# shibiaowan/SHARP

Hardware: AMD Instinct MI355X
Metric: cells/sec end-to-end SHARP (fixed genes, n.RP); ARI vs reference labels (higher is better)
Workload: dtype f64

## Files before the change

### sharp_amd/csrc/common.hpp

```cpp
#pragma once
#include <hip/hip_runtime.h>
#include <functional>

#include <cstdint>
#include <cstdio>
#include <map>
#include <stdexcept>
#include <string>
#include <vector>

#include "../../include/sharp_hip.h"

namespace sharp {

struct Error : std::runtime_error {
    int code;
    Error(int c, const std::string &m) : std::runtime_error(m), code(c) {}
};

void set_error(const std::string &msg);

#define SHARP_HIP_CHECK(expr)                                                                   \
    do {                                                                                        \
        hipError_t _e = (expr);                                                                 \
// ... 37 lines not shown
};

struct Knobs {
    bool rp_dual = true;
    int rp_two_streams = -1;
    int rp_ahead = 2;
    int rp_chunk = 0;
    int rp_cp_wgs = 8;
    int rp_ap_wgs = 4;
    int rp_kernel = 0;
    int rp_pc_wgs = 2;
    int rp_pc_shape = 0;
    int x_storage = 0;
    bool block_prefetch = true;
    bool unlimited_batch = true;
    int unlimited_window_mb = 0;
    int ml_min_levels = 0;
    bool hc_mono = false, hc_seq = false;
    int hc_split = -1;
    int hc_ranges = 0, hc_wpt = 0, hc_finish_at = 15, hc_chunk = 0;
    int tail_threads = 4;
    bool tail_priority = true;
    bool dist_i8 = false;
    bool stats_sums = true;
    bool stats_lane = true;
    bool hc_tri = false;
    bool hc_prep_early = true;
    bool hc_pipe = true;
    bool mean_early = false;
    int gemm_slice = 8;
    bool proj_host = false;
    int hc_front = 0;
    bool hc_nn_gemm = true;
    bool hc_half = false;
    int host_threads = 0;
    int upload_threads = 0;
    std::vector<int> devices;
    int front_overlap = 0;
    int hc_first_chunk = 0;
    int host_group = 1;
    bool decision_log = false;
    bool free_later = true;
    bool step_marks = false;
    int rp_shape = 0;
};
const Knobs &knobs();
void reload_knobs();
// ... 147 lines not shown
```

### sharp_amd/csrc/hclust.hip

```cpp
#include "hclust_task.hpp"

#include <algorithm>
#include <array>
#include <climits>
#include <cmath>
#include <cstring>
#include <limits>

#include "linalg.hpp"

namespace sharp {

namespace {

template <typename T>
struct PinnedBuf {
    T *p = nullptr;
    size_t n = 0;
    PinnedBuf() = default;
    PinnedBuf(const PinnedBuf &) = delete;
    PinnedBuf &operator=(const PinnedBuf &) = delete;
    ~PinnedBuf() { if (p) (void)hipHostFree(p); }
    void ensure(size_t count) {
        if (count <= n) return;
// ... 38 lines not shown
    }
}

inline long long rup(long long v, long long a) { return (v + a - 1) / a * a; }

constexpr int kHcSplitMaxTasks = 136;
constexpr int kMlMinLevels = 256;
static int ml_min_levels() { return knobs().ml_min_levels > 0 ? knobs().ml_min_levels : kMlMinLevels; }
constexpr int kHcSplitMinObs = 1000;

struct ChunkJob {
    size_t i0 = 0, i1 = 0;
    int T = 0, slot = 0;
    bool pipe = false, first = true;
    hipEvent_t input_ready = nullptr;
    bool i8 = false;
    std::vector<HcMeta> metas;
    std::vector<RowPrepTask> prep;
    std::vector<GemmTask> g;
    long long oOut = 0, oM = 0, oLab = 0;
    int max_n = 0, max_p = 0, max_nk = 0, max_kpad = 0, NS = 1;
    bool split = false;
    bool ml = false;
    std::vector<MlMeta> mlmetas;
    int ml_off = 0, ml_cnt = 0, mlt_off = 0, mlt_cnt = 0;
    bool seq_pending = false;
    bool has_next = false;
    bool one_range = false;
    int scratch_slot = 0;
    int prev_slot = 1, next_slot = 1;
    int plan_row = -1;
    int next2_slot = -1;
    hipEvent_t mid_event = nullptr;
    int mid_round = 8;
    bool mid_recorded = false;
    struct Range { int t0, t1; int off[5], cnt[5]; int off8 = 0; bool any_sym, any_feat; };
    std::vector<Range> ranges;
};
enum : int { PH_DIST = 1, PH_AGGLO = 2, PH_STATS = 4, PH_ALL = 7 };
struct PipeEvents {
    hipEvent_t in = nullptr, out[8] = {nullptr}, gemm[6] = {nullptr}, hc[6] = {nullptr}, done[6] = {nullptr}, prep[6] = {nullptr};
};
PipeEvents &pipe_events() {
    PipeEvents &e = per_slot<PipeEvents>();
    if (!e.in) {
        SHARP_HIP_CHECK(hipEventCreateWithFlags(&e.in, hipEventDisableTiming));
// ... 45 lines not shown
            M.kmin = M.kmax = tk.prm.N_cluster;
        } else {
            M.kmin = tk.prm.minN;
            M.kmax = std::min(tk.prm.maxN, tk.n - 1);
            SHARP_REQUIRE(M.kmin >= 2 && M.kmax >= M.kmin, "get_opt_hclust: empty range of cluster numbers (minN.cluster..maxN.cluster)");
        }
        M.nk = M.kmax - M.kmin + 1;
        M.kpad = static_cast<int>(rup(M.kmax, 16));
        M.oD = oD; oD += static_cast<long long>(M.nld) * M.nld;
        M.oD0 = oD0; if (M.symmetric == 1) oD0 += static_cast<long long>(M.nld) * M.nld;
        M.oCr = oCr; if (M.symmetric != 2) oCr += static_cast<long long>(M.n) * M.p;
        M.oCt = oCt; if (M.symmetric != 2) oCt += rup(M.p, 16) * M.nld;
        M.oNrm = oN; oN += M.n;
        M.oM = oM; oM += M.n;
        M.oLab = oLab; oLab += static_cast<long long>(M.nk) * M.n;
        M.oH = M.oT = M.oG = oK; oK += static_cast<long long>(M.nld) * M.kpad;
        M.oCSt = oCS; oCS += static_cast<long long>(M.p) * M.kpad;
        M.oQ = oQ; oQ += static_cast<long long>(M.kpad) * M.kpad;
        M.oOut = oOut; oOut += 2LL * M.nk;
        max_n = std::max(max_n, M.n); max_p = std::max(max_p, M.p); max_nk = std::max(max_nk, M.nk);
        max_kpad = std::max(max_kpad, M.kpad);
    }
    J.oOut = oOut; J.oM = oM; J.oLab = oLab; J.max_n = max_n; J.max_p = max_p; J.max_nk = max_nk; J.max_kpad = max_kpad;
    SHARP_REQUIRE(max_nk > ml_min_levels() ||
                  stats_lds_bytes(max_n, std::max(max_kpad, 64)) <= ST_LDS_MAX,
                  "get_opt_hclust: this many observations with this many candidate cluster numbers does not fit the silhouette kernel "
                  "(LDS: 8 B per observation rounded up to a power of two + 36 B per candidate cluster)");
    { HostTimer ht("hc_workspace_alloc");
    W.D.ensure(oD); W0.S0.ensure(oD); W0.S1.ensure(oD); W.D0.ensure(std::max<long long>(oD0, 1)); W.Cr.ensure(oCr); W.Ct.ensure(oCt); W.nrm.ensure(oN);
    W.height.ensure(oM); W.ia.ensure(oM); W.ib.ensure(oM); W.lab.ensure(oLab);
    W.H.ensure(oK); W.T.ensure(oK); W.G.ensure(oK); W.CSt.ensure(oCS); W.Q.ensure(oQ); W.out.ensure(oOut); }
    { HostTimer ht("hc_workspace_alloc");
    W.meta.ensure(T); W.prep.ensure(T); W.gemm.ensure(5 * static_cast<size_t>(T)); W.status.ensure(T); }
    {
        bool parts = knobs().hc_nn_gemm;
#ifdef SHARP_LAB
        if (knobs().dist_i8 && max_p <= 8192) parts = false;
#endif
        long long oNN = 0;
        if (parts) for (int t = 0; t < T; ++t) if (!metas[t].symmetric && metas[t].nld <= 2048) oNN += static_cast<long long>(metas[t].nld / 128) * metas[t].nld;
        if (oNN > 0) {
            W.nnp.ensure(oNN);
            oNN = 0;
            for (int t = 0; t < T; ++t) if (!metas[t].symmetric && metas[t].nld <= 2048) { metas[t].nn = W.nnp.p + oNN; oNN += static_cast<long long>(metas[t].nld / 128) * metas[t].nld; }
        }
    }
    W.meta.upload(metas.data(), T);

    int NS = T >= 194 ? 2 : 1;
    {
        const bool split = knobs().hc_split >= 0 ? knobs().hc_split == 1 : (T <= kHcSplitMaxTasks && max_n >= kHcSplitMinObs);
        J.split = split;
        if (!knobs().hc_seq && ((!knobs().hc_mono && split) || max_n > HR_MAXN)) NS = 1;
    }
    if (knobs().hc_ranges > 0) NS = std::max(1, std::min(8, knobs().hc_ranges));
    if (J.pipe || J.one_range) NS = 1;
    if (J.max_nk > ml_min_levels()) NS = 1;
    NS = std::min(NS, T);
    std::vector<RowPrepTask> &prep = J.prep;
    prep.assign(T, RowPrepTask());
    for (int t = 0; t < T; ++t) {
        const HcTask &tk = tasks[i0 + t];
        const HcMeta &M = metas[t];
        prep[t] = RowPrepTask{tk.d_mat, tk.ld, M.n, M.p, M.nld, static_cast<int>(rup(M.p, 16)), M.symmetric, W.Cr.p + M.oCr,
                              W.Ct.p + M.oCt, W.nrm.p + M.oNrm, W.D.p + M.oD};
    }
    W.prep.upload(prep.data(), T);
    typedef ChunkJob::Range Range;
    J.NS = NS;
    std::vector<Range> &ranges = J.ranges;
    ranges.assign(NS, Range());
    std::vector<GemmTask> &g = J.g;
    g.clear();
    g.reserve(5 * static_cast<size_t>(T));
    for (int s = 0; s < NS; ++s) {
        Range &R = ranges[s];
        R.t0 = static_cast<int>(static_cast<long long>(T) * s / NS);
        R.t1 = static_cast<int>(static_cast<long long>(T) * (s + 1) / NS);
        R.any_sym = R.any_feat = false;
        for (int kind = 0; kind < 5; ++kind) {
            R.off[kind] = static_cast<int>(g.size());
            for (int t = R.t0; t < R.t1; ++t) {
                const HcMeta &M = metas[t];
                R.any_sym |= M.symmetric != 0; R.any_feat |= M.symmetric == 0;
                switch (kind) {
                    case 0:
                        if (!M.symmetric) g.push_back(GemmTask{W.Ct.p + M.oCt, W.Ct.p + M.oCt, W.D.p + M.oD, M.n, M.n, M.p, M.nld, M.nld, M.nld, 1, 1, 1,
                                                               const_cast<double *>(M.nn), M.method == 8});
                        break;
                    case 1:
                        g.push_back(GemmTask{W.Cr.p + M.oCr, W.H.p + M.oH, W.CSt.p + M.oCSt, M.p, M.kpad, M.n, M.p, M.kpad, M.kpad, 0, 0, 0});
                        break;
                    case 2:
                        g.push_back(GemmTask{W.CSt.p + M.oCSt, W.Ct.p + M.oCt, W.G.p + M.oG, M.kpad, M.n, M.p, M.kpad, M.nld, M.nld, 0, 0, 0});
                        break;
                    case 3:
                        g.push_back(GemmTask{W.CSt.p + M.oCSt, W.CSt.p + M.oCSt, W.Q.p + M.oQ, M.kpad, M.kpad, M.p, M.kpad, M.kpad, M.kpad, 0, 0, 0});
                        break;
                    default:
                        if (M.symmetric == 1) g.push_back(GemmTask{W.H.p + M.oH, W.D0.p + M.oD0, W.T.p + M.oT, M.kpad, M.n, M.n, M.kpad, M.nld, M.nld, 0, 0, 0});
                        break;
                }
            }
            R.cnt[kind] = static_cast<int>(g.size()) - R.off[kind];
        }
    }
#ifdef SHARP_LAB
    J.i8 = knobs().dist_i8 && max_p <= 8192;
    if (J.i8) {
        std::vector<DistI8Task> d8;
        size_t oSl = 0, oSc = 0;
        for (int t = 0; t < T; ++t) if (!metas[t].symmetric) { oSl += dist_i8_slice_bytes(metas[t].nld, metas[t].p); oSc += metas[t].nld; }
        W.sl.ensure(std::max<size_t>(oSl, 1)); W.slscale.ensure(std::max<size_t>(oSc, 1));
        oSl = 0; oSc = 0;
        for (int s = 0; s < NS; ++s) {
            ranges[s].off8 = static_cast<int>(d8.size());
            for (int t = ranges[s].t0; t < ranges[s].t1; ++t) {
                const HcMeta &M = metas[t];
                if (M.symmetric) continue;
                d8.push_back(DistI8Task{W.Cr.p + M.oCr, W.D.p + M.oD, W.sl.p + oSl, W.slscale.p + oSc, M.n, M.p, M.nld, (M.p + 31) / 32});
                oSl += dist_i8_slice_bytes(M.nld, M.p); oSc += M.nld;
            }
        }
        W.i8.ensure(std::max<size_t>(d8.size(), 1));
        if (!d8.empty()) W.i8.upload(d8.data(), d8.size());
    }
#endif
    J.ml = max_nk > ml_min_levels();
    if (J.ml) {
        SHARP_REQUIRE(static_cast<size_t>(max_kpad) * 22 + 64 <= HR_LDS_CU, "get_opt_hclust: too many candidate cluster numbers (more than ~7400)");
        J.ml_off = static_cast<int>(g.size());
        for (int t = 0; t < T; ++t) {
            const HcMeta &M = metas[t];
            g.push_back(GemmTask{W.Ct.p + M.oCt, W.CSt.p + M.oCSt, W.G.p + M.oG, M.n, M.kpad, M.p, M.nld, M.kpad, M.kpad, 0, 0, 0});
        }
        J.ml_cnt = T;
        J.mlt_off = static_cast<int>(g.size());
        for (int t = 0; t < T; ++t) {
            const HcMeta &M = metas[t];
            if (M.symmetric == 1) g.push_back(GemmTask{W.D0.p + M.oD0, W.H.p + M.oH, W.T.p + M.oT, M.n, M.kpad, M.n, M.nld, M.kpad, M.kpad, 0, 0, 0});
        }
        J.mlt_cnt = static_cast<int>(g.size()) - J.mlt_off;
        W.gemm.ensure(g.size());
        J.mlmetas.assign(T, MlMeta());
        long long oS = 0, oMg = 0, oFin = 0;
        for (int t = 0; t < T; ++t) {
            const HcMeta &M = metas[t];
            J.mlmetas[t].oS = oS; oS += 2LL * M.n * M.nk;
            J.mlmetas[t].oMerge = oMg; oMg += M.nk;
            J.mlmetas[t].oFin = oFin; oFin += M.kmax;
        }
// ... 51 lines not shown
        }
        if (phases & PH_AGGLO) {
        if (J.pipe && !J.first) SHARP_HIP_CHECK(hipStreamWaitEvent(st, EV.hc[J.prev_slot], 0));
        {
            const bool use_rnn = !knobs().hc_seq;
            KernelTimer tm("hclust");
            HcAggloDid did;
            if (use_rnn && hclust_bulk_synchronous(agglo, J.split, W0.img, W0.remaining, J.mid_event, J.mid_round, &did)) J.mid_recorded = true;
            if (!use_rnn || !(J.pipe && J.has_next)) launch_sequential(use_rnn);
            else J.seq_pending = true;
            if (J.plan_row >= 0 && s == 0) {
                std::array<int, kHcPlanCols> &row = batch_plan().rows[J.plan_row];
                row[9] = J.seq_pending; row[10] = did.form; row[14] = did.wpt; row[15] = did.finish_at;
            }
        }
        if (J.pipe) SHARP_HIP_CHECK(hipEventRecord(EV.hc[J.slot], st));
        if (J.pipe && knobs().step_marks)
            SHARP_HIP_CHECK(hipLaunchHostFunc(st, [](void *) { step_mark("    (device) an agglomeration ends"); }, nullptr));
        }
        if (!(phases & PH_STATS)) continue;
        if (J.pipe && J.has_next) SHARP_HIP_CHECK(hipStreamWaitEvent(st, EV.gemm[J.next_slot], 0));
        if (J.pipe && J.next2_slot >= 0) SHARP_HIP_CHECK(hipStreamWaitEvent(st, EV.gemm[J.next2_slot], 0));
        if (J.seq_pending) { launch_sequential(true); J.seq_pending = false; }
        const HcStatsRange stats{dmeta, Ts, max_n, max_p, J.max_nk, max_kpad, R.any_sym, W.gemm.p, R.off, R.cnt, W.ia.p, W.ib.p, W.lab.p,
                                 W.H.p, W.Cr.p, W.CSt.p, W.T.p, W.G.p, W.Q.p, W.nrm.p, W.out.p};
        const HcManyLevels many{&J.metas, &J.mlmetas, W.mlmeta.p, J.oM, J.ml_off, J.ml_cnt, J.mlt_off, J.mlt_cnt, W.mlr1.p, W.mlr2.p, W.mlcntF.p,
                                W.mlcn2m.p, W.mlB.p, W.mlcn2F.p, W.mltot2.p, W.mlS.p};
        hclust_level_stats(stats, J.ml ? &many : nullptr);
        if (NS > 1) {
            SHARP_HIP_CHECK(hipEventRecord(ev_out[s], st));
            SHARP_HIP_CHECK(hipStreamWaitEvent(main_stream, ev_out[s], 0));
        }
    }
    if (J.pipe && (phases & PH_STATS)) SHARP_HIP_CHECK(hipEventRecord(EV.done[J.slot], chunk_stream));
    if (J.pipe && (phases & PH_STATS) && knobs().step_marks)
        SHARP_HIP_CHECK(hipLaunchHostFunc(chunk_stream, [](void *) { step_mark("    (device) a chunk's statistics end"); }, nullptr));
}

void finish_chunk(const std::vector<HcTask> &tasks, ChunkJob &J, bool want_v, std::vector<HcResult> &out, bool want_status) {
    Ctx &c = ctx();
    Workspace &W = ws(J.slot);
    const size_t i0 = J.i0;
    const int T = J.T;
    const long long oOut = J.oOut, oM = J.oM, oLab = J.oLab;
    const std::vector<HcMeta> &metas = J.metas;
    if (J.pipe) SHARP_HIP_CHECK(hipStreamWaitEvent(c.stream, pipe_events().done[J.slot], 0));
    W.h_out.ensure(std::max<long long>(oOut, 1)); W.h_height.ensure(std::max<long long>(oM, 1));
    double *h_out = W.h_out.p, *h_height = W.h_height.p;
// ... 476 lines not shown
```

### sharp_amd/csrc/hclust_stats.hip

```cpp
#include "hclust_task.hpp"

#include <algorithm>
#include <vector>

#include "linalg.hpp"

namespace sharp {

__global__ __launch_bounds__(HC_THREADS) void cutree_kernel(const HcMeta *__restrict__ metas, const int *__restrict__ ia_all,
                                                            const int *__restrict__ ib_all, int *__restrict__ lab_all) {
    const HcMeta M = metas[blockIdx.x];
    const int n = M.n;
    const int *ia = ia_all + M.oM, *ib = ib_all + M.oM;
    int *lab = lab_all + M.oLab;
    extern __shared__ __attribute__((aligned(16))) unsigned char sm[];
    unsigned char *lds_cursor = sm;
    CUTREE_ARRAYS(LDS_CARVE, n)
    const int tid = threadIdx.x;
    for (int i = tid; i < n; i += HC_THREADS) { absorbed[i] = 0x7fffffff; parent[i] = static_cast<uint16_t>(i); }
    __syncthreads();
    for (int s = tid; s < n - 1; s += HC_THREADS) { absorbed[ib[s] - 1] = s; parent[ib[s] - 1] = static_cast<uint16_t>(ia[s] - 1); }
    __syncthreads();
    const int chunk = (n + HC_THREADS - 1) / HC_THREADS;
    for (int L = 0; L < M.nk; ++L) {
// ... 50 lines not shown
    const double *Cr = Cr_all + M.oCr;
    const int j = j0 + lane;
    const bool live = j < p;
    double *mine = acc + static_cast<size_t>(wave) * kpad * 64 + lane;
    int i = wave;
    for (; i + 3 * SS_WAVES < n; i += 4 * SS_WAVES) {
        double x[4];
        int c[4];
#pragma unroll
        for (int u = 0; u < 4; ++u) {
            c[u] = __builtin_amdgcn_readfirstlane(lab[i + u * SS_WAVES]) - 1;
            x[u] = live ? Cr[static_cast<long long>(i + u * SS_WAVES) * p + j] : 0.0;
        }
#pragma unroll
        for (int u = 0; u < 4; ++u) mine[c[u] * 64] += x[u];
    }
    for (; i < n; i += SS_WAVES) {
        const int c = __builtin_amdgcn_readfirstlane(lab[i]) - 1;
        mine[c * 64] += live ? Cr[static_cast<long long>(i) * p + j] : 0.0;
    }
    __syncthreads();
    double *CSt = CSt_all + M.oCSt;
    for (int q = tid; q < kpad * 64; q += 64 * SS_WAVES) {
        const int c = q >> 6, l = q & 63;
        if (j0 + l >= p) continue;
        double v = acc[c * 64 + l];
#pragma unroll
        for (int w = 1; w < SS_WAVES; ++w) v += acc[(w * kpad + c) * 64 + l];
        CSt[static_cast<long long>(j0 + l) * kpad + c] = v;
    }
}

__global__ void copy_d_kernel(const HcMeta *__restrict__ metas, const double *__restrict__ Dall, double *__restrict__ D0all) {
    const HcMeta M = metas[blockIdx.y];
    if (M.symmetric != 1) return;
    const long long tot = static_cast<long long>(M.n) * M.nld;
    const double *D = Dall + M.oD;
    double *D0 = D0all + M.oD0;
    for (long long q = blockIdx.x * static_cast<long long>(blockDim.x) + threadIdx.x; q < tot;
         q += static_cast<long long>(gridDim.x) * blockDim.x)
        D0[q] = D[q];
}


__global__ __launch_bounds__(ST_THREADS) void stats_kernel(const HcMeta *__restrict__ metas, const int *__restrict__ lab_all,
                                                           const double *__restrict__ T_all, const double *__restrict__ G_all,
// ... 390 lines not shown
    allow_dynamic_lds(ml_level_kernel, lds_l);
    for (int t = 0; t < T; ++t) {
        const HcMeta &M = metas[t];
        const int blocks = std::min((M.n + ML_WAVES - 1) / ML_WAVES, c.num_cu * std::max(1, static_cast<int>(HR_LDS_CU / std::max<size_t>(lds_c, 1))));
        hipLaunchKernelGGL(ml_cells_kernel, dim3(blocks), dim3(64 * ML_WAVES), lds_c, st, r.metas, ml.dml, t, r.lab, r.T, r.G, r.nrm,
                           ml.r1, ml.r2, ml.cn2m, ml.cntF, ml.cn2F, ml.S);
        hipLaunchKernelGGL(ml_level_kernel, dim3(M.nk), dim3(ST_THREADS), lds_l, st, r.metas, ml.dml, t, ml.S, ml.B, r.out);
    }
    launch_check("ml_cells_kernel");
}

}

void hclust_level_stats(const HcStatsRange &r, const HcManyLevels *ml) {
    hipStream_t st = ctx().stream;
    const int Ts = r.tasks, max_n = r.max_n, max_p = r.max_p, max_nk = r.max_nk, max_kpad = r.max_kpad;
    {
        const size_t lds = cutree_lds_bytes(max_n);
        allow_dynamic_lds(cutree_kernel, lds);
        KernelTimer tm("cutree");
        hipLaunchKernelGGL(cutree_kernel, dim3(Ts), dim3(HC_THREADS), lds, st, r.metas, r.ia, r.ib, r.lab);
        launch_check("cutree_kernel");
    }
    const bool sums = knobs().stats_sums && !ml && max_kpad <= SS_KMAX;
    if (!sums || r.any_sym) {
        KernelTimer tm("onehot");
        hipLaunchKernelGGL(onehot_kernel, dim3(64, Ts), dim3(256), 0, st, r.metas, r.lab, r.H);
        launch_check("onehot_kernel");
    }
    if (sums) {
        KernelTimer tm("cluster_sums_gemm");
        const size_t lds = cluster_sums_lds_bytes(max_kpad);
        allow_dynamic_lds(cluster_sums_kernel, lds);
        hipLaunchKernelGGL(cluster_sums_kernel, dim3((max_p + 63) / 64, Ts), dim3(64 * SS_WAVES), lds, st, r.metas, r.lab, r.Cr, r.CSt);
        launch_check("cluster_sums_kernel");
    } else if (r.cnt[1]) gemm_tn_f64_batched(r.gemm + r.off[1], r.cnt[1], max_p, max_kpad, "cluster_sums_gemm");
    if (ml) { many_levels_stats(r, *ml); return; }
    if (r.cnt[2]) gemm_tn_f64_batched(r.gemm + r.off[2], r.cnt[2], max_kpad, max_n, "row_cluster_dot_gemm");
    if (r.cnt[3]) gemm_tn_f64_batched(r.gemm + r.off[3], r.cnt[3], max_kpad, max_kpad, "cluster_gram_gemm");
    if (r.cnt[4]) gemm_tn_f64_batched(r.gemm + r.off[4], r.cnt[4], max_kpad, max_n, "dist_cluster_sums_gemm");
    const int kcap = std::max(max_kpad, 64);
    const bool lane_form = knobs().stats_lane && max_kpad <= 64;
    const size_t lds = lane_form ? stats_lane_lds_bytes(max_n, kcap) : stats_lds_bytes(max_n, kcap);
    const auto kern = lane_form ? stats_lane_kernel : stats_kernel;
    allow_dynamic_lds(kern, lds);
    KernelTimer tm("sil_ch_stats");
    const long long blocks = static_cast<long long>((Ts + 7) / 8) * 8 * max_nk;
    hipLaunchKernelGGL(kern, dim3(static_cast<unsigned>(blocks)), dim3(ST_THREADS), lds, st, r.metas, r.lab, r.T,
                       r.G, r.Q, r.nrm, r.out, Ts, max_nk, kcap);
    launch_check("stats_kernel");
}

}
// ... 1 lines not shown
```

### sharp_amd/csrc/hclust_task.hpp

```cpp
#pragma once
#include <algorithm>

#include "hclust.hpp"

namespace sharp {

#define SHARP_HC_LOCAL __attribute__((visibility("hidden")))

struct HcMeta {
    int n, p, nld, kmin, kmax, nk, kpad, method;
    int symmetric, pad0;
    long long oD, oD0;
    long long oCr, oCt, oNrm;
    long long oM;
    long long oLab;
    long long oH, oT, oG;
    long long oCSt, oQ;
    long long oOut;
    const double *nn;
};
struct MlMeta {
    long long oS;
    long long oMerge;
    long long oFin;
};

constexpr int HC_THREADS = 512;
constexpr double HC_INF = 1.0e300;
constexpr int HR_MAXN = 4096;
constexpr size_t HR_LDS_CU = 160 * 1024;
constexpr int ST_THREADS = 512;
constexpr size_t ST_LDS_MAX = 160 * 1024;
constexpr int SS_WAVES = 2, SS_KMAX = 144;
constexpr int ML_WAVES = 3;

template <typename K>
static inline void allow_dynamic_lds(K kern, size_t bytes) {
    SHARP_HIP_CHECK(hipFuncSetAttribute(reinterpret_cast<const void *>(kern), hipFuncAttributeMaxDynamicSharedMemorySize, static_cast<int>(bytes)));
}

__host__ __device__ inline int hc_npow2(int n) { int p = 1; while (p < n) p <<= 1; return p; }

#define LDS_CARVE(type, name, count) \
    [[maybe_unused]] type *name = reinterpret_cast<type *>(lds_cursor); lds_cursor = reinterpret_cast<unsigned char *>(name + (count));
#define LDS_COUNT(type, name, count) lds_bytes += sizeof(type) * static_cast<size_t>(count);

#define HC_SEQ_STATE_ARRAYS(X, n, nal)                                                                                      \
    X(double, disnn, nal)                                                                                                   \
    X(double, pv, 32)                                                                                                       \
    X(int, nn, nal)                                                                                                         \
    X(int, membr, nal)                                                                                                      \
    X(int, list, nal)                                                                                                       \
    X(int, pi, 32)                                                                                                          \
    X(int, cnt, 2)                                                                                                          \
    X(unsigned char, flag, n)
#define HC_SEQ_SCRATCH_ARRAYS(X, n)                                                                                         \
// ... 25 lines not shown
    X(int, wsum, (nwave) + 1)                                                                                               \
    X(unsigned char, tie, nal)
inline size_t hr_image_bytes(int max_n) {
    const int nal = (max_n + 3) & ~3;
    size_t lds_bytes = 0;
    HR_STATE_ARRAYS(LDS_COUNT, nal, 1024 / 64)
    const size_t slack = 64;
    return std::max((lds_bytes + slack + 15) / 16 * 16, static_cast<size_t>(hc_npow2(max_n - 1)) * 16);
}

#define CUTREE_ARRAYS(X, n)                                                                                                 \
    X(int, absorbed, n)                                             \
    X(int, wsum, HC_THREADS / 64 + 1)                                                                                       \
    X(uint16_t, parent, n)                                                                      \
    X(uint16_t, rank, n)
inline size_t cutree_lds_bytes(int max_n) {
    size_t lds_bytes = 0;
    CUTREE_ARRAYS(LDS_COUNT, max_n)
    return lds_bytes + 16;
}

inline size_t cluster_sums_lds_bytes(int kpad) { return static_cast<size_t>(SS_WAVES) * kpad * 64 * 8; }

inline size_t stats_lds_bytes(int max_n, int kcap) {
    int npow2 = 1; while (npow2 < max_n) npow2 <<= 1;
    return static_cast<size_t>(npow2) * 8 + ST_THREADS * 8 + 2 * static_cast<size_t>(kcap) * 8 + (5 * static_cast<size_t>(kcap) + 8) * 4;
}

#define ML_PREP_ARRAYS(X, kf)                                                                                               \
    X(double, cn2, kf)                                                                                                      \
    X(double, ctot, kf)                                                                                                     \
    X(double, part, 1024)                                                                                                   \
    X(int, cnt, kf)
inline size_t ml_prep_lds_bytes(int kpad) {
    size_t lds_bytes = 0;
    ML_PREP_ARRAYS(LDS_COUNT, kpad)
    return lds_bytes + 64;
}

#define ML_CELLS_ARRAYS(X, kf)                                                                                              \
    X(double, st, kf)                        \
    X(double, sg, kf)                                                         \
    X(uint16_t, cnt, kf)                                                                                                    \
    X(uint16_t, live, kf)                                                 \
    X(uint16_t, pos, kf)
__host__ __device__ inline size_t ml_cells_wave_bytes(int kf) {
// ... 15 lines not shown

struct HcAggloRange {
    const HcMeta *metas;
    int tasks, max_n;
    double *D, *S0, *S1;
    int *ia, *ib;
    double *height;
    int *status;
};
struct HcAggloDid {
    int form = 0;
    int wpt = 0;
    int finish_at = 0;
};
SHARP_HC_LOCAL bool hclust_bulk_synchronous(const HcAggloRange &r, bool split, DevBuf<unsigned char> &img, DevBuf<int> &remaining,
                                            hipEvent_t mid_event, int mid_round, HcAggloDid *did = nullptr);
SHARP_HC_LOCAL void hclust_sequential(const HcAggloRange &r, const int *only_if, unsigned char *gstate);

struct GemmTask;
struct HcStatsRange {
    const HcMeta *metas;
    int tasks, max_n, max_p, max_nk, max_kpad;
    bool any_sym;
    const GemmTask *gemm;
    const int *off, *cnt;
    const int *ia, *ib;
    int *lab;
    double *H, *Cr, *CSt, *T, *G, *Q, *nrm, *out;
};
struct HcManyLevels {
    const std::vector<HcMeta> *metas;
    const std::vector<MlMeta> *mlmetas;
    const MlMeta *dml;
    long long oM;
    int ml_off, ml_cnt, mlt_off, mlt_cnt;
    int *r1, *r2, *cntF;
    double *cn2m, *B, *cn2F, *tot2, *S;
};
SHARP_HC_LOCAL void hclust_copy_d(const HcMeta *metas, int tasks, const double *D, double *D0);
SHARP_HC_LOCAL void hclust_level_stats(const HcStatsRange &r, const HcManyLevels *ml);
SHARP_HC_LOCAL void hclust_pack_labels(const HcMeta *metas, int tasks, const int *lab, const int *chosen, const long long *dst_off, int *dst);

SHARP_HC_LOCAL void select_level(const HcParams &prm, int n, int nk, const double *msil, const double *CH, const double *height,
                                 int &oind, int &branch, int &rc);
SHARP_HC_LOCAL double host_ch_euclid(const double *y, int n, int p, const int *cl, int g);

}
```

### sharp_amd/csrc/linalg.hip

```cpp
#include "linalg.hpp"
#include "graph.hpp"

#include <algorithm>
#include <cstring>
#include <string>
#include <type_traits>
#include <vector>

namespace sharp {

typedef __attribute__((address_space(1))) const double *gcdp;
typedef __attribute__((address_space(1))) double *gdp;


typedef double v4f64 __attribute__((ext_vector_type(4)));

__device__ __forceinline__ void lds_barrier() { asm volatile("s_waitcnt lgkmcnt(0)\n\ts_barrier" ::: "memory"); }

constexpr int GT = 64, GK = 16, GLD = 80;

__global__ __launch_bounds__(256) void gemm_tn_f64_kernel(const GemmTask *__restrict__ tasks) {
    const GemmTask t = tasks[blockIdx.z];
    const int m0 = blockIdx.y * GT, n0 = blockIdx.x * GT;
    if (m0 >= t.M || n0 >= t.N) return;
// ... 252 lines not shown
    for (int z0 = 0; z0 < count; z0 += 65535) {
        const int nz = std::min(65535, count - z0);
        if (fast) {
            const int ntm = (max_M + FT - 1) / FT, ntn = (max_N + FT - 1) / FT;
            const int tiles_max = symmetric ? ntn * (ntn + 1) / 2 : ntm * ntn;
            const long long blocks = static_cast<long long>((nz + 7) / 8) * 8 * tiles_max;
            long long slice = blocks;
            if (c.polite) {
                const int per_cu = knobs().gemm_slice;
                if (per_cu > 0) slice = static_cast<long long>(c.num_cu) * per_cu;
            }
            for (long long b0 = 0; b0 < blocks; b0 += slice)
                hipLaunchKernelGGL(gemm_tn_f64_fast_kernel, dim3(static_cast<unsigned>(std::min(slice, blocks - b0))), dim3(512), 0, c.stream,
                                   d_tasks + z0, nz, tiles_max, b0);
        }
        else
            hipLaunchKernelGGL(gemm_tn_f64_kernel, dim3((max_N + GT - 1) / GT, (max_M + GT - 1) / GT, nz), dim3(256), 0, c.stream,
                               d_tasks + z0);
        launch_check("gemm_tn_f64_kernel");
    }
}

constexpr int RP_MAXV = 8;

__device__ __forceinline__ bool fused_rows(const RowPrepTask &t) { return t.mode == 0 && t.p <= 64 * RP_MAXV; }

__global__ __launch_bounds__(256) void row_prep_kernel(const RowPrepTask *__restrict__ tasks, int skip_fused) {
    const RowPrepTask t = tasks[blockIdx.y];
    const int lane = threadIdx.x & 63;
    const int row = blockIdx.x * 4 + (threadIdx.x >> 6);
    if (row >= t.n) return;
    gcdp x = (gcdp)t.src + static_cast<long long>(row) * t.lds;
    gdp cr = (gdp)t.Cr + static_cast<long long>(row) * t.p;
    const int p = t.p;
    if (fused_rows(t) && skip_fused) return;
    if (t.mode == 2) {
        gdp drow = (gdp)t.D + static_cast<long long>(row) * t.nld;
        for (int q = lane; q < p; q += 64) drow[q] = q == row ? 0.0 : x[q];
        return;
    }
    if (t.mode == 0 && p <= 64 * RP_MAXV) {
        double xv[RP_MAXV];
#pragma unroll
        for (int u = 0; u < RP_MAXV; ++u) { const int q = lane + 64 * u; xv[u] = x[q < p ? q : 0]; }
        double s = 0.0;
#pragma unroll
// ... 61 lines not shown
    __syncthreads();
    for (int j = ty; j < 32; j += 8) {
        const int q = q0 + j, r = r0 + tx;
        if (q < t.p_pad && r < t.nld) ((gdp)t.Ct)[static_cast<long long>(q) * t.nld + r] = (r < t.n && q < t.p) ? tile[tx][j] : 0.0;
    }
}

constexpr int RT_ROWS = 16;
__global__ __launch_bounds__(256) void row_prep_t_kernel(const RowPrepTask *__restrict__ tasks) {
    const RowPrepTask t = tasks[blockIdx.y];
    const int r0 = blockIdx.x * RT_ROWS;
    if (!fused_rows(t) || r0 >= t.nld) return;
    extern __shared__ double rt_tile[];
    const int p = t.p, ldt = t.p_pad + 1;
    const int lane = threadIdx.x & 63, wave = threadIdx.x >> 6;
    for (int i = wave; i < RT_ROWS; i += 4) {
        const int row = r0 + i;
        double *trow = rt_tile + i * ldt;
        if (row >= t.n) {
            for (int q = lane; q < t.p_pad; q += 64) trow[q] = 0.0;
            continue;
        }
        gcdp x = (gcdp)t.src + static_cast<long long>(row) * t.lds;
        gdp cr = (gdp)t.Cr + static_cast<long long>(row) * t.p;
        double xv[RP_MAXV];
#pragma unroll
        for (int u = 0; u < RP_MAXV; ++u) { const int q = lane + 64 * u; xv[u] = x[q < p ? q : 0]; }
        double s = 0.0;
#pragma unroll
        for (int u = 0; u < RP_MAXV; ++u) if (lane + 64 * u < p) s += xv[u];
        const double mean = wave_sum(s) / p;
        double ss = 0.0;
#pragma unroll
        for (int u = 0; u < RP_MAXV; ++u) if (lane + 64 * u < p) { const double c = xv[u] - mean; ss += c * c; }
        const double sd = sqrt(wave_sum(ss) / static_cast<double>(p - 1 > 1 ? p - 1 : 1));
        double s2 = 0.0;
#pragma unroll
        for (int u = 0; u < RP_MAXV; ++u) if (lane + 64 * u < p) { xv[u] = (xv[u] - mean) / sd; s2 += xv[u]; }
        const double mean2 = wave_sum(s2) / p;
        double n2 = 0.0;
#pragma unroll
        for (int u = 0; u < RP_MAXV; ++u) if (lane + 64 * u < p) { xv[u] -= mean2; n2 += xv[u] * xv[u]; }
        const double nr = sqrt(wave_sum(n2));
#pragma unroll
        for (int u = 0; u < RP_MAXV; ++u) {
            const int q = lane + 64 * u;
            if (q < p) { const double v = xv[u] / nr; cr[q] = v; trow[q] = v; }
            else if (q < t.p_pad) trow[q] = 0.0;
        }
        if (lane == 0) ((gdp)t.nrm)[row] = 1.0;
    }
    __syncthreads();
    const int i = threadIdx.x & (RT_ROWS - 1);
    for (int q = threadIdx.x / RT_ROWS; q < t.p_pad; q += 256 / RT_ROWS)
        ((gdp)t.Ct)[static_cast<long long>(q) * t.nld + r0 + i] = rt_tile[i * ldt + q];
}

void row_prep_batched(const RowPrepTask *d_tasks, int count, int max_n, int max_p, bool all_feature_rows) {
    if (count <= 0 || max_n <= 0) return;
    Ctx &c = ctx();
    KernelTimer tm("row_prep");
    const bool fused = max_p <= 64 * RP_MAXV;
    for (int z0 = 0; z0 < count; z0 += 65535) {
        const int nz = std::min(65535, count - z0);
        const int nld_max = (max_n + 127) / 128 * 128;
        if (fused) {
            const size_t lds = static_cast<size_t>(RT_ROWS) * ((max_p + 15) / 16 * 16 + 1) * sizeof(double);
            SHARP_HIP_CHECK(hipFuncSetAttribute(reinterpret_cast<const void *>(row_prep_t_kernel), hipFuncAttributeMaxDynamicSharedMemorySize,
                                                static_cast<int>(lds)));
            hipLaunchKernelGGL(row_prep_t_kernel, dim3(nld_max / RT_ROWS, nz), dim3(256), lds, c.stream, d_tasks + z0);
// ... 174 lines not shown
```

### sharp_amd/csrc/linalg.hpp

```cpp
#pragma once
#include "common.hpp"

namespace sharp {

struct GemmTask {
    const double *At;
    const double *Bt;
    double *C;
    int M, N, K;
    long long lda, ldb, ldc;
    int epilogue;
    int symmetric;
    int fast;
    double *nn = nullptr;
    int nn_square = 0;
};

void gemm_tn_f64_batched(const GemmTask *d_tasks, int count, int max_M, int max_N, const char *timer_name, bool fast = false,
                         bool symmetric = false);

struct RowPrepTask {
    const double *src;
    long long lds;
    int n, p, nld;
    int p_pad;
    int mode;
    double *Cr;
    double *Ct;
    double *nrm;
    double *D;
};
void row_prep_batched(const RowPrepTask *d_tasks, int count, int max_n, int max_p, bool all_feature_rows = false);


#ifdef SHARP_LAB
constexpr int kDistI8Slices = 7;
struct DistI8Task {
    const double *Cr;
    double *D;
    signed char *sl;
    double *scale;
    int n, p, nld, ksteps;
};
size_t dist_i8_slice_bytes(int nld, int p);
void dist_i8_batched(const DistI8Task *d_tasks, int count, int max_n);
void dist_i8_slices(const DistI8Task *d_tasks, int count, int max_n);
void dist_i8_products(const DistI8Task *d_tasks, int count, int max_n);
#endif

}
```

### sharp_amd/csrc/runtime.hip

```cpp
#include <cstring>
#include <ctime>
#include <atomic>
#include <condition_variable>
#include <exception>
#include <pthread.h>
#include <mutex>
#include <thread>
#include <unistd.h>
#include <sstream>
#include <tuple>
#include <vector>
#include <cstdio>

#include "common.hpp"

namespace sharp {

static thread_local std::string g_last_error;
static thread_local int t_slot = 0;
static Ctx g_ctxs[kMaxSlots];

void set_error(const std::string &msg) { g_last_error = msg; }

int cur_slot() { return t_slot; }
// ... 269 lines not shown
    auto num = [&](const char *name, int dflt) { const char *e = env(name); return e && *e ? atoi(e) : dflt; };
    if (const char *kv = env("SHARP_RP_KERNEL")) v.rp_kernel = !strcmp(kv, "fused") ? 1 : !strcmp(kv, "dense") ? 2 : !strcmp(kv, "pc") ? 4 : 0;
    if (const char *xs = env("SHARP_X_STORAGE")) v.x_storage = !strcmp(xs, "fp32") ? 32 : !strcmp(xs, "fp64") ? 64 : 0;
    v.host_threads = num("SHARP_HOST_THREADS", 0);
    v.upload_threads = num("SHARP_UPLOAD_THREADS", 0);
    v.tail_threads = num("SHARP_TAIL_THREADS", 4);
    v.unlimited_batch = num("SHARP_UNLIMITED_BATCH", 1) != 0;
    v.unlimited_window_mb = num("SHARP_UNLIMITED_WINDOW_MB", 0);
    v.block_prefetch = num("SHARP_NO_BLOCK_PREFETCH", 0) == 0;
    v.decision_log = num("SHARP_DECISION_LOG", 0) != 0;
    v.host_group = num("SHARP_HOST_GROUP", 1);
    v.step_marks = num("SHARP_STEP_MARKS", 0) != 0;
    v.hc_seq = num("SHARP_HC_SEQ", 0) == 1;
    v.hc_mono = num("SHARP_HC_MONO", 0) == 1;
    v.hc_split = num("SHARP_HC_SPLIT", -1);
    v.hc_pipe = num("SHARP_HC_PIPE", 1) != 0;
    v.hc_chunk = num("SHARP_HC_CHUNK", 0);
    v.hc_first_chunk = num("SHARP_HC_FIRST_CHUNK", 0);
    v.hc_ranges = num("SHARP_HC_RANGES", 0);
    v.hc_wpt = num("SHARP_HC_WPT", 0);
    v.hc_finish_at = num("SHARP_HC_FINISH_AT", 15);
    v.hc_nn_gemm = num("SHARP_HC_NN_GEMM", 1) != 0;
    v.stats_lane = num("SHARP_STATS_LANE", 1) != 0;
    v.ml_min_levels = num("SHARP_ML_MIN_LEVELS", 0);
    v.proj_host = num("SHARP_PROJ_HOST", 0) == 1;
    v.rp_pc_wgs = std::max(1, num("SHARP_RP_PC_WGS", 2));
    v.gemm_slice = num("SHARP_GEMM_SLICE", 8);
#ifdef SHARP_LAB
    if (const char *kv = env("SHARP_RP_KERNEL")) { if (!strcmp(kv, "sparse")) v.rp_kernel = 3; else if (!strcmp(kv, "split")) v.rp_kernel = 5; }
    v.rp_dual = num("SHARP_RP_DUAL", 1) != 0;
    { const int ser = num("SHARP_RP_SERIAL", -1); v.rp_two_streams = ser < 0 ? -1 : (ser == 0 ? 1 : 0); }
    v.rp_chunk = num("SHARP_RP_CHUNK", 0);
    v.rp_ahead = num("SHARP_RP_AHEAD", 2);
    v.rp_cp_wgs = std::max(1, num("SHARP_RP_CP_WGS", 8));
    v.rp_ap_wgs = std::max(1, num("SHARP_RP_AP_WGS", 4));
    v.rp_shape = num("SHARP_RP_SHAPE", 0);
    if (const char *ps = env("SHARP_RP_PC_SHAPE")) v.rp_pc_shape = (*ps == 'a' || *ps == 'A') ? 1 : (*ps == 'b' || *ps == 'B') ? 2 : 0;
    v.mean_early = num("SHARP_MEAN_EARLY", 0) != 0;
    v.hc_prep_early = num("SHARP_HC_PREP_EARLY", 1) != 0;
    v.hc_tri = num("SHARP_HC_TRI", 0) != 0;
    v.hc_front = num("SHARP_HC_FRONT", 0);
    v.hc_half = num("SHARP_HC_HALF", 0) != 0;
    v.stats_sums = num("SHARP_STATS_SUMS", 1) != 0;
    v.dist_i8 = num("SHARP_DIST_I8", 0) != 0;
    v.free_later = num("SHARP_FREE_LATER", 1) != 0;
    v.front_overlap = num("SHARP_FRONT_OVERLAP", 0);
    v.tail_priority = num("SHARP_TAIL_PRIORITY", 1) != 0;
#endif
    if (const char *dl = env("SHARP_DEVICES")) {
        for (const char *q = dl; *q;) {
            char *end = nullptr;
            const long dvc = strtol(q, &end, 10);
            if (end == q) break;
            v.devices.push_back(static_cast<int>(dvc));
            q = *end == ',' ? end + 1 : end;
        }
    }
    return v;
}
static Knobs &knobs_storage() { static Knobs k = read_knobs(); return k; }
const Knobs &knobs() { return knobs_storage(); }
void reload_knobs() { knobs_storage() = read_knobs(); }

namespace {
struct StepMarks { std::mutex mu; std::vector<std::tuple<const char *, int, double>> v; };
StepMarks &step_marks() { static StepMarks *M = new StepMarks; return *M; }
// ... 211 lines not shown
```

Measured before the change: 3.170 million.

## Compute cluster sums from transposed Ct and drop the Cr row buffer

Adds a cluster-sums kernel that reads the transposed normalized matrix Ct through a register-prefetched LDS tile, instead of reading the row-major Cr copy. When no other consumer needs Cr (non-symmetric, small p), row prep no longer writes Cr and its workspace is not allocated. The aim is to cut one full matrix write and its memory footprint. The cost is a more complex kernel with LDS carving and a per-label conditional accumulation that may be slower than the previous reduction.

```diff
diff --git a/sharp_amd/csrc/common.hpp b/sharp_amd/csrc/common.hpp
--- a/sharp_amd/csrc/common.hpp
+++ b/sharp_amd/csrc/common.hpp
@@ -83,7 +83,7 @@
     int tail_threads = 4;
     bool tail_priority = true;
     bool dist_i8 = false;
-    bool stats_sums = true;
+    int stats_sums = 1;
     bool stats_lane = true;
     bool hc_tri = false;
     bool hc_prep_early = true;
diff --git a/sharp_amd/csrc/hclust.hip b/sharp_amd/csrc/hclust.hip
--- a/sharp_amd/csrc/hclust.hip
+++ b/sharp_amd/csrc/hclust.hip
@@ -84,6 +84,8 @@
     int max_n = 0, max_p = 0, max_nk = 0, max_kpad = 0, NS = 1;
     bool split = false;
     bool ml = false;
+    int sums_form = SUMS_CT;
+    bool keep_cr = true;
     std::vector<MlMeta> mlmetas;
     int ml_off = 0, ml_cnt = 0, mlt_off = 0, mlt_cnt = 0;
     bool seq_pending = false;
@@ -175,12 +177,20 @@
         max_kpad = std::max(max_kpad, M.kpad);
     }
     J.oOut = oOut; J.oM = oM; J.oLab = oLab; J.max_n = max_n; J.max_p = max_p; J.max_nk = max_nk; J.max_kpad = max_kpad;
+    J.ml = max_nk > ml_min_levels();
+    J.sums_form = cluster_sums_form(knobs().stats_sums, J.ml, max_n, max_kpad);
+    J.keep_cr = J.sums_form != SUMS_CT;
+    for (const HcMeta &M : metas) J.keep_cr |= M.symmetric != 0 || M.p > kRowPrepFusedMaxP;
+#ifdef SHARP_LAB
+    J.keep_cr |= knobs().dist_i8 && max_p <= 8192;
+#endif
+    if (!J.keep_cr) { oCr = 0; for (HcMeta &M : metas) M.oCr = 0; }
     SHARP_REQUIRE(max_nk > ml_min_levels() ||
                   stats_lds_bytes(max_n, std::max(max_kpad, 64)) <= ST_LDS_MAX,
                   "get_opt_hclust: this many observations with this many candidate cluster numbers does not fit the silhouette kernel "
                   "(LDS: 8 B per observation rounded up to a power of two + 36 B per candidate cluster)");
     { HostTimer ht("hc_workspace_alloc");
-    W.D.ensure(oD); W0.S0.ensure(oD); W0.S1.ensure(oD); W.D0.ensure(std::max<long long>(oD0, 1)); W.Cr.ensure(oCr); W.Ct.ensure(oCt); W.nrm.ensure(oN);
+    W.D.ensure(oD); W0.S0.ensure(oD); W0.S1.ensure(oD); W.D0.ensure(std::max<long long>(oD0, 1)); if (J.keep_cr) W.Cr.ensure(oCr); W.Ct.ensure(oCt); W.nrm.ensure(oN);
     W.height.ensure(oM); W.ia.ensure(oM); W.ib.ensure(oM); W.lab.ensure(oLab);
     W.H.ensure(oK); W.T.ensure(oK); W.G.ensure(oK); W.CSt.ensure(oCS); W.Q.ensure(oQ); W.out.ensure(oOut); }
     { HostTimer ht("hc_workspace_alloc");
@@ -212,10 +222,11 @@
     NS = std::min(NS, T);
     std::vector<RowPrepTask> &prep = J.prep;
     prep.assign(T, RowPrepTask());
+    double *const Cr = J.keep_cr ? W.Cr.p : nullptr;
     for (int t = 0; t < T; ++t) {
         const HcTask &tk = tasks[i0 + t];
         const HcMeta &M = metas[t];
-        prep[t] = RowPrepTask{tk.d_mat, tk.ld, M.n, M.p, M.nld, static_cast<int>(rup(M.p, 16)), M.symmetric, W.Cr.p + M.oCr,
+        prep[t] = RowPrepTask{tk.d_mat, tk.ld, M.n, M.p, M.nld, static_cast<int>(rup(M.p, 16)), M.symmetric, Cr ? Cr + M.oCr : nullptr,
                               W.Ct.p + M.oCt, W.nrm.p + M.oNrm, W.D.p + M.oD};
     }
     W.prep.upload(prep.data(), T);
@@ -242,7 +253,7 @@
                                                                const_cast<double *>(M.nn), M.method == 8});
                         break;
                     case 1:
-                        g.push_back(GemmTask{W.Cr.p + M.oCr, W.H.p + M.oH, W.CSt.p + M.oCSt, M.p, M.kpad, M.n, M.p, M.kpad, M.kpad, 0, 0, 0});
+                        g.push_back(GemmTask{Cr ? Cr + M.oCr : nullptr, W.H.p + M.oH, W.CSt.p + M.oCSt, M.p, M.kpad, M.n, M.p, M.kpad, M.kpad, 0, 0, 0});
                         break;
                     case 2:
                         g.push_back(GemmTask{W.CSt.p + M.oCSt, W.Ct.p + M.oCt, W.G.p + M.oG, M.kpad, M.n, M.p, M.kpad, M.nld, M.nld, 0, 0, 0});
@@ -279,7 +290,6 @@
         if (!d8.empty()) W.i8.upload(d8.data(), d8.size());
     }
 #endif
-    J.ml = max_nk > ml_min_levels();
     if (J.ml) {
         SHARP_REQUIRE(static_cast<size_t>(max_kpad) * 22 + 64 <= HR_LDS_CU, "get_opt_hclust: too many candidate cluster numbers (more than ~7400)");
         J.ml_off = static_cast<int>(g.size());
@@ -377,8 +387,8 @@
         if (J.pipe && J.has_next) SHARP_HIP_CHECK(hipStreamWaitEvent(st, EV.gemm[J.next_slot], 0));
         if (J.pipe && J.next2_slot >= 0) SHARP_HIP_CHECK(hipStreamWaitEvent(st, EV.gemm[J.next2_slot], 0));
         if (J.seq_pending) { launch_sequential(true); J.seq_pending = false; }
-        const HcStatsRange stats{dmeta, Ts, max_n, max_p, J.max_nk, max_kpad, R.any_sym, W.gemm.p, R.off, R.cnt, W.ia.p, W.ib.p, W.lab.p,
-                                 W.H.p, W.Cr.p, W.CSt.p, W.T.p, W.G.p, W.Q.p, W.nrm.p, W.out.p};
+        const HcStatsRange stats{dmeta, Ts, max_n, max_p, J.max_nk, max_kpad, R.any_sym, J.sums_form, W.gemm.p, R.off, R.cnt, W.ia.p, W.ib.p, W.lab.p,
+                                 W.H.p, J.keep_cr ? W.Cr.p : nullptr, W.Ct.p, W.CSt.p, W.T.p, W.G.p, W.Q.p, W.nrm.p, W.out.p};
         const HcManyLevels many{&J.metas, &J.mlmetas, W.mlmeta.p, J.oM, J.ml_off, J.ml_cnt, J.mlt_off, J.mlt_cnt, W.mlr1.p, W.mlr2.p, W.mlcntF.p,
                                 W.mlcn2m.p, W.mlB.p, W.mlcn2F.p, W.mltot2.p, W.mlS.p};
         hclust_level_stats(stats, J.ml ? &many : nullptr);
diff --git a/sharp_amd/csrc/hclust_stats.hip b/sharp_amd/csrc/hclust_stats.hip
--- a/sharp_amd/csrc/hclust_stats.hip
+++ b/sharp_amd/csrc/hclust_stats.hip
@@ -96,6 +96,77 @@
     __syncthreads();
     double *CSt = CSt_all + M.oCSt;
     for (int q = tid; q < kpad * 64; q += 64 * SS_WAVES) {
+        const int c = q >> 6, l = q & 63;
+        if (j0 + l >= p) continue;
+        double v = acc[c * 64 + l];
+#pragma unroll
+        for (int w = 1; w < SS_WAVES; ++w) v += acc[(w * kpad + c) * 64 + l];
+        CSt[static_cast<long long>(j0 + l) * kpad + c] = v;
+    }
+}
+
+__device__ __forceinline__ void sc_lds_barrier() { asm volatile("s_waitcnt lgkmcnt(0)\n\ts_barrier" ::: "memory"); }
+
+typedef double sc_v2f64 __attribute__((ext_vector_type(2)));
+__global__ __launch_bounds__(SC_THREADS) void cluster_sums_ct_kernel(const HcMeta *__restrict__ metas, const int *__restrict__ lab_all,
+                                                                     const double *__restrict__ Ct_all, double *__restrict__ CSt_all) {
+    static_assert(SS_WAVES == 2 && SC_THREADS == 256 && SC_TI == 32 && SS_KMAX <= 256, "the thread maps below");
+    const HcMeta M = metas[blockIdx.y];
+    const int j0 = blockIdx.x * 64;
+    if (j0 >= M.p) return;
+    const int kpad = M.kpad, n = M.n, p = M.p;
+    extern __shared__ __attribute__((aligned(16))) unsigned char sc_sm[];
+    unsigned char *lds_cursor = sc_sm;
+    CLUSTER_SUMS_CT_ARRAYS(LDS_CARVE, kpad, n)
+    const int tid = threadIdx.x, lane = tid & 63;
+    const int wave = __builtin_amdgcn_readfirstlane(tid >> 6);
+    for (int q = tid; q < SS_WAVES * kpad * 64; q += SC_THREADS) acc[q] = 0.0;
+    const int *lab = lab_all + M.oLab + static_cast<long long>(M.nk - 1) * n;
+    for (int i = tid; i < n; i += SC_THREADS) labs[i] = static_cast<unsigned char>(lab[i] - 1);
+    const int ip = tid & 15, jr = tid >> 4;
+    const int ntiles = (n + SC_TI - 1) / SC_TI;
+    const double *Ct = Ct_all + M.oCt + static_cast<long long>(j0 + jr) * M.nld + 2 * ip;
+    const long long row16 = 16LL * M.nld;
+    sc_v2f64 buf[SC_DEPTH][4];
+    auto fetch = [&](sc_v2f64 (&b)[4], int t) {
+#pragma unroll
+        for (int u = 0; u < 4; ++u) {
+            const bool in = t < ntiles && j0 + jr + 16 * u < p;
+            b[u] = in ? *reinterpret_cast<const sc_v2f64 *>(Ct + u * row16 + t * SC_TI) : sc_v2f64{0.0, 0.0};
+        }
+    };
+#pragma unroll
+    for (int d = 0; d < SC_DEPTH; ++d) fetch(buf[d], d);
+    const int cls = wave & 1, csel = wave >> 1;
+    double *mine = acc + static_cast<size_t>(cls) * kpad * 64 + lane;
+    for (int t0 = 0; t0 < ntiles; t0 += SC_DEPTH) {
+#pragma unroll
+        for (int d = 0; d < SC_DEPTH; ++d) {
+            const int t = t0 + d;
+            if (t >= ntiles) break;
+#pragma unroll
+            for (int u = 0; u < 4; ++u) {
+                tile[(2 * ip) * SC_LDT + jr + 16 * u] = buf[d][u].x;
+                tile[(2 * ip + 1) * SC_LDT + jr + 16 * u] = buf[d][u].y;
+            }
+            fetch(buf[d], t + SC_DEPTH);
+            sc_lds_barrier();
+            double x[SC_TI / 2];
+            int c[SC_TI / 2];
+#pragma unroll
+            for (int u = 0; u < SC_TI / 2; ++u) {
+                const int ii = cls + 2 * u, i = t * SC_TI + ii;
+                x[u] = tile[ii * SC_LDT + lane];
+                c[u] = i < n ? __builtin_amdgcn_readfirstlane(static_cast<int>(labs[i])) : -1;
+            }
+#pragma unroll
+            for (int u = 0; u < SC_TI / 2; ++u)
+                if (c[u] >= 0 && (c[u] & 1) == csel) mine[c[u] * 64] += x[u];
+            sc_lds_barrier();
+        }
+    }
+    double *CSt = CSt_all + M.oCSt;
+    for (int q = tid; q < kpad * 64; q += SC_THREADS) {
         const int c = q >> 6, l = q & 63;
         if (j0 + l >= p) continue;
         double v = acc[c * 64 + l];
@@ -532,13 +603,19 @@
         hipLaunchKernelGGL(cutree_kernel, dim3(Ts), dim3(HC_THREADS), lds, st, r.metas, r.ia, r.ib, r.lab);
         launch_check("cutree_kernel");
     }
-    const bool sums = knobs().stats_sums && !ml && max_kpad <= SS_KMAX;
+    const bool sums = r.sums_form != SUMS_GEMM;
     if (!sums || r.any_sym) {
         KernelTimer tm("onehot");
         hipLaunchKernelGGL(onehot_kernel, dim3(64, Ts), dim3(256), 0, st, r.metas, r.lab, r.H);
         launch_check("onehot_kernel");
     }
-    if (sums) {
+    if (r.sums_form == SUMS_CT) {
+        KernelTimer tm("cluster_sums_gemm");
+        const size_t lds = cluster_sums_ct_lds_bytes(max_kpad, max_n);
+        allow_dynamic_lds(cluster_sums_ct_kernel, lds);
+        hipLaunchKernelGGL(cluster_sums_ct_kernel, dim3((max_p + 63) / 64, Ts), dim3(SC_THREADS), lds, st, r.metas, r.lab, r.Ct, r.CSt);
+        launch_check("cluster_sums_ct_kernel");
+    } else if (sums) {
         KernelTimer tm("cluster_sums_gemm");
         const size_t lds = cluster_sums_lds_bytes(max_kpad);
         allow_dynamic_lds(cluster_sums_kernel, lds);
diff --git a/sharp_amd/csrc/hclust_task.hpp b/sharp_amd/csrc/hclust_task.hpp
--- a/sharp_amd/csrc/hclust_task.hpp
+++ b/sharp_amd/csrc/hclust_task.hpp
@@ -32,6 +32,7 @@
 constexpr int ST_THREADS = 512;
 constexpr size_t ST_LDS_MAX = 160 * 1024;
 constexpr int SS_WAVES = 2, SS_KMAX = 144;
+constexpr int SC_THREADS = 256, SC_TI = 32, SC_DEPTH = 4, SC_LDT = 65;
 constexpr int ML_WAVES = 3;
 
 template <typename K>
@@ -103,6 +104,23 @@
 
 inline size_t cluster_sums_lds_bytes(int kpad) { return static_cast<size_t>(SS_WAVES) * kpad * 64 * 8; }
 
+#define CLUSTER_SUMS_CT_ARRAYS(X, kpad, n)                                                                                  \
+    X(double, acc, SS_WAVES * (kpad) * 64)                                                    \
+    X(double, tile, SC_TI * SC_LDT)                                           \
+    X(unsigned char, labs, ((n) + 15) & ~15)
+inline size_t cluster_sums_ct_lds_bytes(int max_kpad, int max_n) {
+    size_t lds_bytes = 0;
+    CLUSTER_SUMS_CT_ARRAYS(LDS_COUNT, max_kpad, max_n)
+    return lds_bytes;
+}
+
+enum : int { SUMS_GEMM = 0, SUMS_CT = 1, SUMS_CR = 2 };
+inline int cluster_sums_form(int knob, bool many_levels, int max_n, int max_kpad) {
+    if (knob == 0 || many_levels || max_kpad > SS_KMAX) return SUMS_GEMM;
+    if (knob == 2 || cluster_sums_ct_lds_bytes(max_kpad, max_n) > HR_LDS_CU) return SUMS_CR;
+    return SUMS_CT;
+}
+
 inline size_t stats_lds_bytes(int max_n, int kcap) {
     int npow2 = 1; while (npow2 < max_n) npow2 <<= 1;
     return static_cast<size_t>(npow2) * 8 + ST_THREADS * 8 + 2 * static_cast<size_t>(kcap) * 8 + (5 * static_cast<size_t>(kcap) + 8) * 4;
@@ -164,11 +182,12 @@
     const HcMeta *metas;
     int tasks, max_n, max_p, max_nk, max_kpad;
     bool any_sym;
+    int sums_form;
     const GemmTask *gemm;
     const int *off, *cnt;
     const int *ia, *ib;
     int *lab;
-    double *H, *Cr, *CSt, *T, *G, *Q, *nrm, *out;
+    double *H, *Cr, *Ct, *CSt, *T, *G, *Q, *nrm, *out;
 };
 struct HcManyLevels {
     const std::vector<HcMeta> *metas;
diff --git a/sharp_amd/csrc/linalg.hip b/sharp_amd/csrc/linalg.hip
--- a/sharp_amd/csrc/linalg.hip
+++ b/sharp_amd/csrc/linalg.hip
@@ -298,6 +298,7 @@
 }
 
 constexpr int RP_MAXV = 8;
+static_assert(64 * RP_MAXV == kRowPrepFusedMaxP, "linalg.hpp tells the callers which rows need no Cr");
 
 __device__ __forceinline__ bool fused_rows(const RowPrepTask &t) { return t.mode == 0 && t.p <= 64 * RP_MAXV; }
 
@@ -405,6 +406,7 @@
             continue;
         }
         gcdp x = (gcdp)t.src + static_cast<long long>(row) * t.lds;
+        const bool keep_cr = t.Cr != nullptr;
         gdp cr = (gdp)t.Cr + static_cast<long long>(row) * t.p;
         double xv[RP_MAXV];
 #pragma unroll
@@ -428,7 +430,7 @@
 #pragma unroll
         for (int u = 0; u < RP_MAXV; ++u) {
             const int q = lane + 64 * u;
-            if (q < p) { const double v = xv[u] / nr; cr[q] = v; trow[q] = v; }
+            if (q < p) { const double v = xv[u] / nr; if (keep_cr) cr[q] = v; trow[q] = v; }
             else if (q < t.p_pad) trow[q] = 0.0;
         }
         if (lane == 0) ((gdp)t.nrm)[row] = 1.0;
diff --git a/sharp_amd/csrc/linalg.hpp b/sharp_amd/csrc/linalg.hpp
--- a/sharp_amd/csrc/linalg.hpp
+++ b/sharp_amd/csrc/linalg.hpp
@@ -30,6 +30,7 @@
     double *nrm;
     double *D;
 };
+constexpr int kRowPrepFusedMaxP = 512;
 void row_prep_batched(const RowPrepTask *d_tasks, int count, int max_n, int max_p, bool all_feature_rows = false);
 
 
diff --git a/sharp_amd/csrc/runtime.hip b/sharp_amd/csrc/runtime.hip
--- a/sharp_amd/csrc/runtime.hip
+++ b/sharp_amd/csrc/runtime.hip
@@ -315,6 +315,7 @@
     v.hc_finish_at = num("SHARP_HC_FINISH_AT", 15);
     v.hc_nn_gemm = num("SHARP_HC_NN_GEMM", 1) != 0;
     v.stats_lane = num("SHARP_STATS_LANE", 1) != 0;
+    { const int ss = num("SHARP_STATS_SUMS", 1); v.stats_sums = ss == 0 || ss == 2 ? ss : 1; }
     v.ml_min_levels = num("SHARP_ML_MIN_LEVELS", 0);
     v.proj_host = num("SHARP_PROJ_HOST", 0) == 1;
     v.rp_pc_wgs = std::max(1, num("SHARP_RP_PC_WGS", 2));
@@ -334,7 +335,6 @@
     v.hc_tri = num("SHARP_HC_TRI", 0) != 0;
     v.hc_front = num("SHARP_HC_FRONT", 0);
     v.hc_half = num("SHARP_HC_HALF", 0) != 0;
-    v.stats_sums = num("SHARP_STATS_SUMS", 1) != 0;
     v.dist_i8 = num("SHARP_DIST_I8", 0) != 0;
     v.free_later = num("SHARP_FREE_LATER", 1) != 0;
     v.front_overlap = num("SHARP_FRONT_OVERLAP", 0);
```

Result: no change. 3.225 million (median of 6 runs) (+1.7%).
